# pandekan/tomography_alignment

Measured on AMD Instinct MI355X. Metric: sirt_iterations_per_sec, higher is better.
Workload: dtype f32

## Files before the change

### tomography_alignment_amd/csrc/kernels_tile_gather.hip.h

```cpp

#define GTX 8
#define GTY 8
#define GROWS 14
#define GPITCH 68
#ifndef GWAVES
#define GWAVES 4
#endif
#ifndef GPX
#define GPX 8
#define GPY 12
#endif

#define G_DPP(V, CTRL) __builtin_amdgcn_update_dpp(0, (V), (CTRL), 0xf, 0xf, true)
__device__ __forceinline__ int gwave_min_i32(int v)
{
    v = min(v, G_DPP(v, 0xB1));
    v = min(v, G_DPP(v, 0x4E));
    v = min(v, G_DPP(v, 0x141));
    v = min(v, G_DPP(v, 0x140));
    return min(min(__builtin_amdgcn_readlane(v, 0), __builtin_amdgcn_readlane(v, 16)), min(__builtin_amdgcn_readlane(v, 32), __builtin_amdgcn_readlane(v, 48)));
}
__device__ __forceinline__ int gwave_max_i32(int v)
{
    v = max(v, G_DPP(v, 0xB1));
// ... 54 lines not shown
    for (int c = threadIdx.x; c < n_chunk; c += 64) {
        bool any = false;
        for (int i = max(0, 64 * c - zc_hi - 1); i <= min(ndz - 1, 64 * c + 63 - zc_lo) && !any; ++i) any = flags[i] != 0;
        if (any) first = min(first, c);
    }
#pragma unroll
    for (int o = 32; o > 0; o >>= 1) first = min(first, __shfl_xor(first, o, 64));
    if (threadIdx.x == 0) *shift = first >= n_chunk ? 0 : (GWAVES - first % GWAVES) % GWAVES;
}

template <bool ZERO>
__device__ __forceinline__ void gather_update_store(float *__restrict__ dst, const float *__restrict__ vv, const float *__restrict__ gt, const f32x2 (&acc2)[32],
                                                    int z0, int nz, int positivity, double *__restrict__ err_out)
{
    double err = 0.0;
#define G_UPD1(R, A, V, G)                                  \
    {                                                       \
        float pr_ = (A) * (V);                              \
        asm volatile("" : "+v"(pr_));        \
        R = R + pr_;                                        \
        if (positivity && R < 0.f) R = 0.f;                 \
        if (gt) { const float e_ = (G) - R; err += (double)e_ * (double)e_; } \
    }
    if (z0 + 64 <= nz && (nz & 3) == 0) {
#pragma unroll
        for (int p = 0; p < 64; p += 4) {
            float4 r = *(float4 *)(dst + p);
            const float4 v = *(const float4 *)(vv + p);
            float4 t = {0.f, 0.f, 0.f, 0.f};
            if (gt) t = *(const float4 *)(gt + p);
            G_UPD1(r.x, ZERO ? 0.f : acc2[p / 2].x, v.x, t.x)
            G_UPD1(r.y, ZERO ? 0.f : acc2[p / 2].y, v.y, t.y)
            G_UPD1(r.z, ZERO ? 0.f : acc2[p / 2 + 1].x, v.z, t.z)
            G_UPD1(r.w, ZERO ? 0.f : acc2[p / 2 + 1].y, v.w, t.w)
            *(float4 *)(dst + p) = r;
            __builtin_amdgcn_sched_barrier(0);
        }
    } else {
#pragma unroll
        for (int p = 0; p < 64; ++p)
            if (z0 + p < nz) {
                float r = dst[p];
                G_UPD1(r, ZERO ? 0.f : ((p & 1) ? acc2[p / 2].y : acc2[p / 2].x), vv[p], gt[p])
                dst[p] = r;
            }
    }
#undef G_UPD1
    if (gt) {
        err = wave_sum_d(err);
        if ((threadIdx.x & 63) == 0) atomicAdd(err_out, err);
    }
}

template <int NJ, int UPD>
__global__ __launch_bounds__(GWAVES * 64, 16 / GWAVES) void k_adj_gather_flat(const GfC *__restrict__ cs, int n_proj, const float *__restrict__ proj,
                                                                 float *__restrict__ vol, TomoGeomC g, int xs, int xe, int patched,
                                                                 const unsigned char *__restrict__ zflags, int zc_lo, int zc_hi, const int *__restrict__ zshift,
                                                                 const float *__restrict__ upd_v, const float *__restrict__ upd_gt, int positivity,
                                                                 double *__restrict__ upd_err)
{
    __shared__ __attribute__((aligned(16))) float rows[GWAVES][GROWS * GPITCH];
    __shared__ float4 wtab[3][GWAVES][64];
    const int lane = threadIdx.x & 63;
    const int wv = __builtin_amdgcn_readfirstlane(threadIdx.x >> 6);
    const int ntx = (xe - xs + GTX - 1) / GTX, nty = (g.ny + GTY - 1) / GTY, nzq = (g.nz + 64 * GWAVES - 1) / (64 * GWAVES) + 1;
    int tx, ty, zq;
    if (patched) {
        const int npx = (ntx + GPX - 1) / GPX, npy = (nty + GPY - 1) / GPY;
        const int slot = (int)(blockIdx.x >> 3), patch = (slot / (GPX * GPY)) * 8 + (int)(blockIdx.x & 7), within = slot % (GPX * GPY);
        const int pxy = patch % (npx * npy);
        zq = patch / (npx * npy);
        tx = (pxy / npy) * GPX + within / GPY;
        ty = (pxy % npy) * GPY + within % GPY;
    } else {
        zq = (int)(blockIdx.x % (unsigned)nzq);
        ty = (int)((blockIdx.x / (unsigned)nzq) % (unsigned)nty);
        tx = (int)(blockIdx.x / ((unsigned)nzq * (unsigned)nty));
    }
    const int x0 = xs + tx * GTX, y0 = ty * GTY, z0 = (zq * GWAVES + wv - *zshift) * 64;
    if (tx >= ntx || ty >= nty || zq >= nzq) return;
    bool zlive = z0 >= 0 && z0 < g.nz;
    if (zlive) {
        bool any = false;
        for (int i = z0 - zc_hi - 1 + lane; i <= z0 + 63 - zc_lo; i += 64) any |= i >= 0 && i < g.ndz && zflags[i] != 0;
        zlive = __builtin_amdgcn_ballot_w64(any) != 0;
    }
    __shared__ int wlive[GWAVES];
    if (lane == 0) wlive[wv] = zlive ? 1 : 0;
    __syncthreads();
    int nl = 0, rk = 0;
#pragma unroll
    for (int w = 0; w < GWAVES; ++w) { nl += wlive[w]; rk += w < wv ? wlive[w] : 0; }
#if !defined(__gfx950__) && !defined(__gfx942__) && !defined(__gfx90a__) && defined(__HIP_DEVICE_COMPILE__)
#error "k_adj_gather_flat: divergent exit before barriers is only known to be safe on gfx9-family targets (s_barrier ignores ended waves)"
#endif
    if (UPD && !zlive && z0 >= 0 && z0 < g.nz && (positivity || upd_gt)) {
        const int X = x0 + (lane >> 3), Y = y0 + (lane & 7);
        if (X < xe && Y < g.ny) {
            const size_t o = ((size_t)X * g.ny + Y) * g.nz + z0;
            f32x2 none[32];
            gather_update_store<true>(vol + o, upd_v + o, upd_gt ? upd_gt + o : nullptr, none, z0, g.nz, positivity, upd_err);
        }
    }
    if (!zlive) return;
    const int X = x0 + (lane >> 3), Y = y0 + (lane & 7), Zl = z0 + lane;
    float *wrows = rows[wv];
    const size_t n_det = (size_t)g.ndx * g.ndz;
    const uint32_t pitch4 = (uint32_t)g.ndz * 4u;
    const float two_m32 = 2.3283064365386963e-10f;
    f32x2 acc2[32];
#pragma unroll
    for (int p = 0; p < 32; ++p) acc2[p] = f32x2{0.f, 0.f};

#define G_TABLE(IPX, BUF, SLOT)                                                                                            \
    {                                                                                                                      \
        float4 t4 = {0.f, 0.f, 0.f, 0.f};                                                                                  \
        if ((IPX) < n_proj) {                                                                                              \
            const GfC &ct = cs[IPX];                                                                                       \
            const float qx = (float)X - ct.p0x, qy = (float)Y - ct.p0y;                                                    \
            const float a = ct.m00 * qx + ct.m01 * qy, b = ct.m10 * qx + ct.m11 * qy;                                      \
            const int i0 = (int)ceilf(a - (fabsf(ct.m00) + fabsf(ct.m01) + 5e-3f));                                        \
            const int j0 = (int)ceilf(b - (fabsf(ct.m10) + fabsf(ct.m11) + 5e-3f));                                        \
            int64_t rx = ct.fp0x + (int64_t)i0 * ct.fux + (int64_t)j0 * ct.fdx - ((int64_t)X << 32);                       \
            int64_t ry = ct.fp0y + (int64_t)i0 * ct.fuy + (int64_t)j0 * ct.fdy - ((int64_t)Y << 32);                       \
            float W[3];                                                                                                    \
            _Pragma("unroll") for (int k = 0; k < 3; ++k) {                                                                \
                int64_t sx = rx, sy = ry;                                                                                  \
                float wsum = 0.f;                                                                                          \
                _Pragma("unroll") for (int mth = 0; mth < NJ; ++mth) {                                                     \
                    const int hx = (int)(sx >> 32), hy = (int)(sy >> 32);                                                  \
                    const float fx = (float)(unsigned)sx * two_m32, fy = (float)(unsigned)sy * two_m32;                    \
                                                        \
                    const float wx = select_lanes2(select_lanes(fx, __builtin_amdgcn_ballot_w64(hx == -1)), 1.f - fx, __builtin_amdgcn_ballot_w64(hx == 0)); \
                    const float wy = select_lanes2(select_lanes(fy, __builtin_amdgcn_ballot_w64(hy == -1)), 1.f - fy, __builtin_amdgcn_ballot_w64(hy == 0)); \
                    wsum += select_lanes(wx * wy, __builtin_amdgcn_ballot_w64((unsigned)(j0 + mth) < (unsigned)ct.n));     \
                    sx += ct.fdx; sy += ct.fdy;                                                                            \
                }                                                                                                          \
                W[k] = select_lanes(wsum, __builtin_amdgcn_ballot_w64((unsigned)(i0 + k) < (unsigned)g.ndx));              \
                rx += ct.fux; ry += ct.fuy;                                                                                \
            }                                                                                                              \
            t4.x = __builtin_bit_cast(float, i0); t4.y = W[0]; t4.z = W[1]; t4.w = W[2];                                   \
        }                                                                                                                  \
        wtab[BUF][SLOT][lane] = t4;                                                                                        \
    }
#ifdef TOMO_ABLATE_GATHER_LOADS
#define G_ROW_LOAD(RS, VOFF, SOFF) __int_as_float(0x3f800000 + (int)((VOFF) + (SOFF)))
#else
#define G_ROW_LOAD(RS, VOFF, SOFF) __builtin_bit_cast(float, __builtin_amdgcn_raw_buffer_load_b32((RS), (VOFF), (SOFF), 0))
#endif
    const uint32_t det_bytes = (uint32_t)min((unsigned long long)n_det * 4ull, 0xffffffffull);
#define G_SETUP(IPX, BUF, SLOT)                                                                                            \
    {                                                                                                                      \
        tn = wtab[BUF][SLOT][lane];                                                                                        \
        hit_n = G_HIT(tn);                                                \
        const int i0s = __builtin_bit_cast(int, tn.x);                                                                     \
        ix_lo_n = __builtin_amdgcn_readfirstlane(gwave_min_i32(i0s));                                                      \
        const GfC &cn = cs[IPX];                                                                                           \
        const int iz0 = Zl - cn.zc;                                                                                        \
        const __amdgpu_buffer_rsrc_t srs =                                                                                 \
            __builtin_amdgcn_make_buffer_rsrc((void *)(proj + (size_t)cn.slot * n_det), 0, (int)det_bytes, 0x00020000);    \
        const uint32_t o0 = (uint32_t)min(max(iz0, 0), g.ndz - 1) * 4u;                                                    \
        const uint32_t rowoff = (uint32_t)min(max(ix_lo_n + min(lane, GROWS - 1), 0), g.ndx - 1) * pitch4;                 \
        _Pragma("unroll") for (int r = 0; r < GROWS; ++r)                                                                  \
            y0v[r] = G_ROW_LOAD(srs, o0, (uint32_t)__builtin_amdgcn_readlane((int)rowoff, r));                             \
         \
         \
        if (cn.tau != 0.f) {                                                 \
            const uint32_t oe = (uint32_t)min(max(z0 - cn.zc - 1, 0), g.ndz - 1) * 4u;                                     \
            yedge = __builtin_bit_cast(float, __builtin_amdgcn_raw_buffer_load_b32(srs, rowoff + oe, 0, 0));               \
        }                                                                                                                  \
    }
#define G_ZLERP(MASKED, TAU)                                                                                                      \
    _Pragma("unroll") for (int r = 0; r < GROWS; ++r) {                                                                           \
        float y1 = dpp_shr1_f(y0v[r]);                                             \
        asm("v_writelane_b32 %0, %1, 0" : "+v"(y1) : "s"(__builtin_amdgcn_readlane(__builtin_bit_cast(int, yedge), r)));    \
        const float a0 = (MASKED) ? select_lanes(y0v[r], m0) : y0v[r], a1 = (MASKED) ? select_lanes(y1, m1) : y1;                \
        wrows[r * GPITCH + lane] = fmaf((TAU), a1 - a0, a0);                                                                      \
    }
#define G_STAGE(IPX)                                                                                                       \
    {                                                                                                                      \
        const GfC &cn = cs[IPX];                                                                                           \
        const int iz0 = Zl - cn.zc, iz1 = iz0 - 1;                                                                         \
        const unsigned long long m0 = __builtin_amdgcn_ballot_w64(iz0 >= 0) & __builtin_amdgcn_ballot_w64(iz0 < g.ndz);    \
        const unsigned long long m1 = __builtin_amdgcn_ballot_w64(iz1 >= 0) & __builtin_amdgcn_ballot_w64(iz1 < g.ndz);    \
        if (cn.tau == 0.f) {             \
            if (m0 == ~0ull) {           \
                _Pragma("unroll") for (int r = 0; r < GROWS; ++r) wrows[r * GPITCH + lane] = y0v[r];     \
            } else {                                                                                                       \
                _Pragma("unroll") for (int r = 0; r < GROWS; ++r) wrows[r * GPITCH + lane] = select_lanes(y0v[r], m0);     \
            }                                                                                                              \
        }                                                                                                                  \
        else if ((m0 & m1) == ~0ull) { G_ZLERP(false, cn.tau) }      \
        else { G_ZLERP(true, cn.tau) }                                                                                     \
    }
#define G_HIT(T) (__any((T).y != 0.f || (T).z != 0.f || (T).w != 0.f))
    const int n_grp = (n_proj + nl - 1) / nl;
    int buf = 0;
    float4 t = {0.f, 0.f, 0.f, 0.f};
    int ix_lo = 0;
    bool hit = false;
    if (n_grp > 0) {
        G_TABLE(rk, 0, rk)
        __syncthreads();
        float4 tn;
        int ix_lo_n = 0;
        bool hit_n;
        float y0v[GROWS], yedge = 0.f;
        G_SETUP(0, 0, 0)
        hit = hit_n;
        if (hit) G_STAGE(0)
        t = tn; ix_lo = ix_lo_n;
    }
    for (int grp = 0; grp < n_grp; ++grp) {
        const int nbuf = buf == 2 ? 0 : buf + 1;
        if (grp + 1 < n_grp) G_TABLE((grp + 1) * nl + rk, nbuf, rk)
        __syncthreads();
        const int g0 = grp * nl, g1 = min(n_proj, g0 + nl);
        for (int ip = g0; ip < g1; ++ip) {
            float4 tn = t;
            int ix_lo_n = ix_lo;
            bool hit_n = false;
            float y0v[GROWS], yedge = 0.f;
            const bool more = ip + 1 < n_proj;
            if (more) {
                const bool same = ip + 1 < g1;
                const int sbuf = same ? buf : nbuf, sslot = same ? ip + 1 - g0 : 0;
                G_SETUP(ip + 1, sbuf, sslot)
            }
            if (hit) {
                const int i0 = __builtin_bit_cast(int, t.x);
                const float W0 = t.y, W1 = t.z, W2 = t.w;
                const int slot0 = min(max(i0 - ix_lo, 0), GROWS - 3);
                const float4 *q = (const float4 *)__builtin_assume_aligned(wrows + slot0 * GPITCH, 16);
                float4 n0 = q[0], n1 = q[GPITCH / 4], n2 = q[2 * GPITCH / 4];
#pragma unroll
                for (int p = 0; p < 64; p += 4) {
                    const float4 r0 = n0, r1 = n1, r2 = n2;
                    if (p + 4 < 64) { n0 = q[(p + 4) / 4]; n1 = q[(GPITCH + p + 4) / 4]; n2 = q[(2 * GPITCH + p + 4) / 4]; }
                    acc2[p / 2] = W2 * f32x2{r2.x, r2.y} + (W1 * f32x2{r1.x, r1.y} + (W0 * f32x2{r0.x, r0.y} + acc2[p / 2]));
                    acc2[p / 2 + 1] = W2 * f32x2{r2.z, r2.w} + (W1 * f32x2{r1.z, r1.w} + (W0 * f32x2{r0.z, r0.w} + acc2[p / 2 + 1]));
                    __builtin_amdgcn_sched_barrier(0);
                }
            }
            hit = hit_n;
            if (hit) G_STAGE(ip + 1)
            t = tn; ix_lo = ix_lo_n;
        }
        buf = nbuf;
    }
#undef G_TABLE
#undef G_ROW_LOAD
#undef G_SETUP
#undef G_ZLERP
#undef G_STAGE
#undef G_HIT
    if (UPD) {
        if (X < xe && Y < g.ny) {
            const size_t o = ((size_t)X * g.ny + Y) * g.nz + z0;
            gather_update_store<false>(vol + o, upd_v + o, upd_gt ? upd_gt + o : nullptr, acc2, z0, g.nz, positivity, upd_err);
        }
    } else if (zlive && X < xe && Y < g.ny) {
        float *dst = vol + ((size_t)X * g.ny + Y) * g.nz + z0;
        if (z0 + 64 <= g.nz && (g.nz & 3) == 0) {
#pragma unroll
            for (int p = 0; p < 64; p += 4) {
                float4 v = *(float4 *)(dst + p);
                v.x += acc2[p / 2].x; v.y += acc2[p / 2].y; v.z += acc2[p / 2 + 1].x; v.w += acc2[p / 2 + 1].y;
                *(float4 *)(dst + p) = v;
            }
        } else {
#pragma unroll
            for (int p = 0; p < 64; ++p)
                if (z0 + p < g.nz) dst[p] += (p & 1) ? acc2[p / 2].y : acc2[p / 2].x;
        }
    }
}


#define FGROWS 24
#define FG_NONE (1 << 29)
#ifndef FPG
#define FPG 16
#define FPR 4
#endif
#define FWD_PATCH_MIN 128

__host__ __device__ static inline unsigned long long fg_list_wgs(int n_list, int nrt, int nzq, int patched)
{
    const unsigned long long npg = (unsigned long long)((n_list + 7) / 8);
    if (!patched) return 8ull * ((npg * (unsigned long long)nrt + 7) / 8) * (unsigned long long)nzq;
    const unsigned long long npq = ((npg + FPG - 1) / FPG) * (unsigned long long)((nrt + FPR - 1) / FPR);
    return 8ull * ((npq * (unsigned long long)nzq + 7) / 8) * (unsigned long long)(FPG * FPR);
}

template <int NW, int WALKY>
__device__ __forceinline__ void fwd_gather_flat_body(const GfC *__restrict__ cs, const int *__restrict__ perm, int n_list, unsigned block_id,
                                                     int patched, float *__restrict__ proj, const float *__restrict__ vol, const TomoGeomC &g,
                                                     const unsigned char *__restrict__ vflags, const int *__restrict__ zshift,
                                                     float (*rows)[FGROWS * GPITCH], float4 (*wtab)[GWAVES][64], int (*ltab)[GWAVES][64], int *wlive)
{
    static_assert(NW == 3 || NW == 4, "NW");
    constexpr int SW = FGROWS - NW + 1;
// ... 281 lines not shown
```

### tomography_alignment_amd/csrc/tomo_ctx.h

```cpp
#ifndef TOMO_CTX_H_
#define TOMO_CTX_H_
#include <hip/hip_runtime.h>
#include <rccl/rccl.h>

#include <deque>
#include <map>
#include <string>
#include <vector>

#include "../../include/tomo.h"
#include "tomo_raycore.h"

struct BpC {
    float rp[3][3], ra[3][3], rb[3][3];
    float t[3];
};

struct ProfRec { int64_t n = 0; double ms = 0.0; };
struct ProfPending { std::string name; hipEvent_t e0, e1; };

struct TilePlan {
    bool valid = false;
    bool ok = false;
    std::vector<double> poses;
    int opts = 0;
    double weight_bound = 2.0;
    int n_flat = 0, n_gather = 0;
    double eb_max = 0.0;
    int zc_lo = 0, zc_hi = 0;
    size_t gf_off = 0, fg_off = 0;
    int fg_n[4] = {0, 0, 0, 0};
    bool fg_ok = false;
};

struct ZfKey {
    const void *src = nullptr;
    int nproj = 0, ndz = 0, ndx = 0, nz = 0, zc_lo = 0, zc_hi = 0;
    bool operator==(const ZfKey &o) const
    {
        return src == o.src && nproj == o.nproj && ndz == o.ndz && ndx == o.ndx && nz == o.nz && zc_lo == o.zc_lo && zc_hi == o.zc_hi;
    }
};

struct tomo_ctx {
    int device = 0;
    hipStream_t stream = nullptr;
    bool has_geom = false;
    TomoGeomC g{};
    double vox_pitch[3] = {1, 1, 1};
    float *d_volpad = nullptr;
    size_t volpad_elems = 0;
    size_t volpad_rows = 0;
    bool halo_dirty = true;
    bool wide_rows = false;
    const void *staged_src = nullptr;
    int reuse_staged = 0;
    void *h_stage = nullptr;
    void *d_stage = nullptr;
    size_t stage_bytes = 0;
    TilePlan plan;
    double *d_red = nullptr;
    double *h_red = nullptr;
    size_t red_cap = 0;
    int comm_test_copy_eighths = 0, comm_test_copy_wgs = 0;
    void *d_comm_scratch = nullptr;
    size_t comm_scratch_bytes = 0;
    double *d_red_part = nullptr;
    size_t red_part_cap = 0;
    double *d_acc = nullptr;
    double *h_acc = nullptr;
    int *d_blk = nullptr;
    size_t blk_ints = 0;
    int reuse_sino_flags = 0;
    ZfKey zf_key;
    bool zf_has_cum = false, zf_has_shift = false;
    bool zf_recorded = false;
    float *d_ws = nullptr;
    size_t ws_elems = 0;
    void *csr_data = nullptr, *csr_indices = nullptr, *csr_indptr = nullptr;
    int64_t csr_nnz = 0, csr_rows = 0;
    int csr_value_bytes = 4;
    int fwd_variant = 3;
    int adj_variant = 2;
    int grad_variant = 4;
    int grad_v1_prec = 0;
    int tile_flat = 1;
    int fused_update = 1;
    int adj_flat_gather = 1;
    int fwd_gather_patch = 1;
    int fwd_flat_gather = 1;
    int fwd_flat_ztiles = 2;
    hipEvent_t ev0 = nullptr, ev1 = nullptr;
    bool profile_on = false;
    std::map<std::string, ProfRec> prof;
    std::vector<ProfPending> pending;
    std::vector<hipEvent_t> ev_pool;
    ncclComm_t comm = nullptr;
    hipStream_t comm_stream = nullptr;
    hipEvent_t ev_compute = nullptr, ev_comm = nullptr;
    bool comm_pending = false;
    std::deque<hipEvent_t> comm_done;
    std::deque<hipEvent_t> comm_done_g;
    int comm_test_poison_us = 0;
    std::vector<hipEvent_t> comm_ev_pool;
    int n_ranks = 1, rank = 0;
    std::string err;
};

int tomo_fail(tomo_ctx *ctx, int code, const std::string &msg);

struct TomoRange {
    bool on;
    explicit TomoRange(const char *name);
    ~TomoRange();
    TomoRange(const TomoRange &) = delete;
    TomoRange &operator=(const TomoRange &) = delete;
};
int tomo_roctx_enable(int on);
int tomo_ensure_stage(tomo_ctx *ctx, size_t bytes);
int tomo_ensure_red(tomo_ctx *ctx, size_t n_doubles);
int tomo_ensure_red_part(tomo_ctx *ctx, size_t n_doubles);
int tomo_ensure_ws(tomo_ctx *ctx, size_t n_floats);
int tomo_ensure_blk(tomo_ctx *ctx, size_t n_ints);
struct BlkHead {
    unsigned char *zf;
    int *zcum, *zshift;
    size_t ints;
};
static inline int tomo_blk_head(tomo_ctx *ctx, size_t extra_ints, BlkHead *h)
{
    const size_t zf_ints = ((size_t)ctx->g.ndz + 3) / 4;
    h->ints = zf_ints + (size_t)ctx->g.ndz + 2;
    const int rc = tomo_ensure_blk(ctx, h->ints + extra_ints);
    if (rc) return rc;
    h->zf = (unsigned char *)ctx->d_blk;
    h->zcum = ctx->d_blk + zf_ints;
    h->zshift = h->zcum + ctx->g.ndz + 1;
    return TOMO_OK;
}
struct LiveList {
    int *list;
// ... 40 lines not shown
```

### tomography_alignment_amd/csrc/tomo_ctx.hip

```cpp
#include <string.h>

#include <algorithm>

#include "tomo_ctx.h"

static std::string g_last_error;

int tomo_fail(tomo_ctx *ctx, int code, const std::string &msg)
{
    g_last_error = msg;
    if (ctx) ctx->err = msg;
    return code;
}

extern "C" int tomo_abi_version(void) { return TOMO_ABI_VERSION; }

extern "C" const char *tomo_last_error(const tomo_ctx *ctx) { return ctx ? ctx->err.c_str() : g_last_error.c_str(); }

extern "C" int tomo_device_count(int *n)
{
    if (!n) return tomo_fail(nullptr, TOMO_ERR_ARG, "null n");
    TOMO_HIP(nullptr, hipGetDeviceCount(n));
    return TOMO_OK;
}
// ... 112 lines not shown
}

extern "C" int tomo_sync(tomo_ctx *ctx)
{
    if (!ctx) return tomo_fail(ctx, TOMO_ERR_ARG, "null ctx");
    TOMO_HIP(ctx, hipStreamSynchronize(ctx->stream));
    return TOMO_OK;
}

extern "C" int tomo_ctx_make_current(tomo_ctx *ctx)
{
    if (!ctx) return tomo_fail(ctx, TOMO_ERR_ARG, "null ctx");
    TOMO_HIP(ctx, hipSetDevice(ctx->device));
    return TOMO_OK;
}

extern "C" int tomo_ctx_stream(tomo_ctx *ctx, void **stream)
{
    if (!ctx || !stream) return tomo_fail(ctx, TOMO_ERR_ARG, "tomo_ctx_stream: null argument");
    *stream = reinterpret_cast<void *>(ctx->stream);
    return TOMO_OK;
}

extern "C" int tomo_ctx_set_cu_mask(tomo_ctx *ctx, const uint32_t *mask, int n_words)
{
    if (!ctx || n_words < 0 || (n_words > 0 && !mask)) return tomo_fail(ctx, TOMO_ERR_ARG, "tomo_ctx_set_cu_mask: bad args");
    if (n_words > 0) {
        bool any = false;
        for (int i = 0; i < n_words; ++i) any |= mask[i] != 0;
        if (!any) return tomo_fail(ctx, TOMO_ERR_ARG, "tomo_ctx_set_cu_mask: empty mask (n_words = 0 restores the unrestricted stream)");
    }
    TOMO_HIP(ctx, hipSetDevice(ctx->device));
    TOMO_HIP(ctx, hipStreamSynchronize(ctx->stream));
    hipStream_t s = nullptr;
    if (n_words == 0) TOMO_HIP(ctx, hipStreamCreateWithFlags(&s, hipStreamNonBlocking));
    else TOMO_HIP(ctx, hipExtStreamCreateWithCUMask(&s, (uint32_t)n_words, mask));
    (void)hipStreamDestroy(ctx->stream);
    ctx->stream = s;
    return TOMO_OK;
}

extern "C" int tomo_set_option(tomo_ctx *ctx, const char *key, int value)
{
    if (!ctx || !key) return tomo_fail(ctx, TOMO_ERR_ARG, "bad args");
    if (!strcmp(key, "fwd_variant")) ctx->fwd_variant = value;
    else if (!strcmp(key, "adj_variant")) ctx->adj_variant = value;
    else if (!strcmp(key, "tile_flat")) ctx->tile_flat = value;
    else if (!strcmp(key, "grad_variant")) ctx->grad_variant = value;
    else if (!strcmp(key, "grad_v1_prec")) ctx->grad_v1_prec = value & 3;
    else if (!strcmp(key, "comm_test_poison_us")) ctx->comm_test_poison_us = value;
    else if (!strcmp(key, "comm_test_copy_eighths")) ctx->comm_test_copy_eighths = value < 0 ? 0 : value;
    else if (!strcmp(key, "comm_test_copy_wgs")) ctx->comm_test_copy_wgs = value < 0 ? 0 : value;
    else if (!strcmp(key, "adj_flat_gather")) ctx->adj_flat_gather = value;
    else if (!strcmp(key, "fused_update")) ctx->fused_update = value;
    else if (!strcmp(key, "fwd_flat_ztiles")) ctx->fwd_flat_ztiles = value;
    else if (!strcmp(key, "fwd_flat_gather")) ctx->fwd_flat_gather = value;
    else if (!strcmp(key, "fwd_gather_patch")) {
        if (value < 0 || value > 2) return tomo_fail(ctx, TOMO_ERR_ARG, "fwd_gather_patch: 0, 1 or 2");
        ctx->fwd_gather_patch = value;
    }
    else if (!strcmp(key, "reuse_staged_volume")) ctx->reuse_staged = value;
    else if (!strcmp(key, "reuse_sino_flags")) ctx->reuse_sino_flags = value;
    else if (!strcmp(key, "roctx")) {
        if (tomo_roctx_enable(value)) return tomo_fail(ctx, TOMO_ERR_UNSUPPORTED, "roctx: neither librocprofiler-sdk-roctx.so nor libroctx64.so could be loaded");
    }
    else return tomo_fail(ctx, TOMO_ERR_ARG, std::string("unknown option ") + key);
    return TOMO_OK;
}

int tomo_ensure_stage(tomo_ctx *ctx, size_t bytes)
{
    ctx->plan.valid = false;
    if (bytes <= ctx->stage_bytes) return TOMO_OK;
    TOMO_HIP(ctx, hipStreamSynchronize(ctx->stream));
    if (ctx->d_stage) (void)hipFree(ctx->d_stage);
    if (ctx->h_stage) (void)hipHostFree(ctx->h_stage);
    ctx->d_stage = ctx->h_stage = nullptr;
    ctx->stage_bytes = 0;
    size_t cap = std::max<size_t>(bytes, 1 << 16);
    TOMO_HIP(ctx, hipMalloc(&ctx->d_stage, cap));
    TOMO_HIP(ctx, hipHostMalloc(&ctx->h_stage, cap, hipHostMallocDefault));
    ctx->stage_bytes = cap;
    return TOMO_OK;
}

int tomo_ensure_red(tomo_ctx *ctx, size_t n)
{
    if (n <= ctx->red_cap) return TOMO_OK;
    TOMO_HIP(ctx, hipStreamSynchronize(ctx->stream));
    if (ctx->d_red) (void)hipFree(ctx->d_red);
    if (ctx->h_red) (void)hipHostFree(ctx->h_red);
    ctx->d_red = ctx->h_red = nullptr;
    ctx->red_cap = 0;
    size_t cap = std::max<size_t>(n, 4096);
    TOMO_HIP(ctx, hipMalloc((void **)&ctx->d_red, cap * sizeof(double)));
    TOMO_HIP(ctx, hipHostMalloc((void **)&ctx->h_red, cap * sizeof(double), hipHostMallocDefault));
    ctx->red_cap = cap;
    return TOMO_OK;
}

int tomo_ensure_red_part(tomo_ctx *ctx, size_t n)
{
    if (n <= ctx->red_part_cap) return TOMO_OK;
    TOMO_HIP(ctx, hipStreamSynchronize(ctx->stream));
    if (ctx->d_red_part) (void)hipFree(ctx->d_red_part);
    ctx->d_red_part = nullptr;
// ... 761 lines not shown
```

### tomography_alignment_amd/csrc/tomo_project.hip

```cpp
#include <limits.h>
#include <string.h>

#include <algorithm>
#include <climits>
#include <vector>

#include "tomo_ctx.h"

#include "kernels_ray.hip.h"
#include "kernels_tile.hip.h"
#include "kernels_tile_flat.hip.h"
#include "kernels_tile_gather.hip.h"
#include "kernels_grad.hip.h"

static inline bool grad_pose_is_tilted(const ProjC &c) { return fabs(c.w[0]) + fabs(c.w[1]) > 0.0157; }

static int upload_projc(tomo_ctx *ctx, const double *h_poses, int n, bool with_grad, ProjC **d_pc, GradC **d_gc,
                        const int32_t *h_rows = nullptr, int *n_first = nullptr)
{
    const size_t pc_bytes = sizeof(ProjC) * (size_t)n;
    const size_t gc_off = (pc_bytes + 255) & ~(size_t)255;
    const size_t total = gc_off + (with_grad ? sizeof(GradC) * (size_t)n : 0);
    TOMO_HIP(ctx, hipStreamSynchronize(ctx->stream));
    int rc = tomo_ensure_stage(ctx, total);
// ... 77 lines not shown
    std::vector<int> fg_list[4];
    p.fg_ok = true;
    p.zc_lo = INT_MAX;
    p.zc_hi = INT_MIN;
    for (int i = 0; i < n_proj; ++i) {
        ProjC pc;
        tomo_make_projc(g, h_poses + (size_t)i * TOMO_POSE_STRIDE, pc, nullptr);
        AdjC a;
        double m[3][3], det = 0.0;
        bool fits = true;
        for (int r = 0; r < 3; ++r) {
            a.p0[r] = pc.p0[r]; a.u[r] = pc.u[r]; a.w[r] = pc.w[r]; a.d[r] = pc.d[r];
            m[r][0] = pc.u[r]; m[r][1] = pc.w[r]; m[r][2] = pc.d[r];
            const double lim = 1073741824.0;
            fits = fits && fabs(pc.p0[r]) < lim && fabs(pc.u[r]) * g.ndx < lim && fabs(pc.w[r]) * g.ndz < lim && fabs(pc.d[r]) * pc.n < lim;
            a.fp0[r] = llround(pc.p0[r] * 4294967296.0);
            a.fu[r] = llround(pc.u[r] * 4294967296.0);
            a.fw[r] = llround(pc.w[r] * 4294967296.0);
            a.fd[r] = llround(pc.d[r] * 4294967296.0);
        }
        a.n = pc.n;
        a.slot = i;
        if (!fits) return TOMO_OK;
        if (!invert3(m, a.minv, &det)) return TOMO_OK;
        if (!(pc.w[2] > 0.7 * sqrt(pc.w[0] * pc.w[0] + pc.w[1] * pc.w[1] + pc.w[2] * pc.w[2]))) return TOMO_OK;
        p.weight_bound = std::max(p.weight_bound, 2.0 / fabs(det));
        const bool untilted = a.fw[0] == 0 && a.fw[1] == 0 && a.fw[2] == ((int64_t)1 << 32) && a.fu[2] == 0 && a.fd[2] == 0 &&
                              ctx->tile_flat != 0;
        const double ea = fabs(a.minv[0][0]) + fabs(a.minv[0][1]), eb = fabs(a.minv[2][0]) + fabs(a.minv[2][1]);
        const bool gatherable = untilted && ctx->adj_flat_gather != 0 && ea < 1.45 && eb < 2.99 &&
                                fabs(a.minv[0][2]) < 1e-9 && fabs(a.minv[2][2]) < 1e-9;
        if (gatherable) {
            GfC q;
            q.fp0x = a.fp0[0]; q.fp0y = a.fp0[1]; q.fux = a.fu[0]; q.fuy = a.fu[1]; q.fdx = a.fd[0]; q.fdy = a.fd[1];
            q.m00 = (float)a.minv[0][0]; q.m01 = (float)a.minv[0][1]; q.m10 = (float)a.minv[2][0]; q.m11 = (float)a.minv[2][1];
            q.p0x = (float)a.p0[0]; q.p0y = (float)a.p0[1];
            q.zc = (int32_t)(a.fp0[2] >> 32);
            q.tau = (float)((double)(uint32_t)(a.fp0[2] & 0xffffffffll) / 4294967296.0);
            q.n = a.n; q.slot = a.slot;
            {
                const bool walky = llabs(q.fdx) < llabs(q.fdy);
                const int64_t ads = llabs(walky ? q.fdy : q.fdx), adl = llabs(walky ? q.fdx : q.fdy);
                p.fg_ok = p.fg_ok && (double)ads >= 0.67 * 4294967296.0 && (double)adl < 0.999 * 4294967296.0;
                std::vector<int> &fl = fg_list[2 * (walky ? 1 : 0) + (2 * adl <= ads ? 0 : 1)];
                if (!fl.empty() && fl.back() != (int)gfc.size() - 1)
                    while (fl.size() % 8) fl.push_back(-1);
                fl.push_back((int)gfc.size());
            }
            gath.push_back(a);
            gfc.push_back(q);
            p.eb_max = std::max(p.eb_max, eb);
            p.zc_lo = std::min(p.zc_lo, (int)q.zc);
            p.zc_hi = std::max(p.zc_hi, (int)q.zc);
        } else
            (untilted ? flat : gen).push_back(a);
    }
    AdjC *h = (AdjC *)ctx->h_stage;
    size_t k = 0;
    for (const AdjC &a : gath) h[k++] = a;
    for (const AdjC &a : flat) h[k++] = a;
    for (const AdjC &a : gen) h[k++] = a;
    GfC *hg = (GfC *)((char *)ctx->h_stage + p.gf_off);
    for (size_t i = 0; i < gfc.size(); ++i) hg[i] = gfc[i];
    int *hf = (int *)((char *)ctx->h_stage + p.fg_off);
    size_t fg_total = 0;
    for (int l = 0; l < 4; ++l) {
        for (int v : fg_list[l]) hf[fg_total++] = v;
        p.fg_n[l] = (int)fg_list[l].size();
    }
    if (n_proj) TOMO_HIP(ctx, hipMemcpyAsync(ctx->d_stage, h, p.fg_off + sizeof(int) * fg_total, hipMemcpyHostToDevice, ctx->stream));
    p.n_gather = (int)gath.size();
    p.n_flat = (int)(gath.size() + flat.size());
    p.poses.assign(h_poses, h_poses + n_pose_doubles);
    p.opts = opts;
    p.ok = p.valid = true;
    return TOMO_OK;
}

static inline const AdjC *plan_adjc(const tomo_ctx *ctx) { return (const AdjC *)ctx->d_stage; }
static inline const GfC *plan_gfc(const tomo_ctx *ctx, const TilePlan &p) { return (const GfC *)((const char *)ctx->d_stage + p.gf_off); }
static inline const int *plan_fwd_lists(const tomo_ctx *ctx, const TilePlan &p) { return (const int *)((const char *)ctx->d_stage + p.fg_off); }

static inline dim3 tile_grid(const TomoGeomC &g, int tz = ATZ) { return dim3((g.nz + 1 + tz - 1) / tz, (g.ny + 1 + ATY - 1) / ATY, (g.nx + 1 + ATX - 1) / ATX); }

static int forward_tiles(tomo_ctx *ctx, const double *h_poses, int n_proj, const float *d_vol, float *d_proj, int xt0, int xt1, bool *done,
                         bool whole = false)
{
    const TomoGeomC &g = ctx->g;
    *done = false;
    if (ctx->fwd_variant != 3 || n_proj <= 0) return TOMO_OK;
    dim3 grid = tile_grid(g);
    if (grid.y > 65535 || grid.z > 65535) return TOMO_OK;
    const TilePlan *plan = nullptr;
    int rc = stage_tile_consts(ctx, h_poses, n_proj, &plan);
    if (rc) return rc;
    if (!plan->ok) return TOMO_OK;
    *done = true;
    xt0 = std::max(xt0, 0);
    xt1 = std::min(xt1, (int)grid.z);
    if (xt1 <= xt0) return TOMO_OK;
    grid.z = (unsigned)(xt1 - xt0);
    const AdjC *d_c = plan_adjc(ctx);
    const int n_flat = plan->n_flat;
    size_t flat_ints = 0;
    ctx->zf_key.src = nullptr;
    if (whole && ctx->fwd_flat_gather && plan->n_gather == n_proj && plan->fg_ok && plan->eb_max < 1.49 &&
// ... 145 lines not shown

static int adjoint_tiles(tomo_ctx *ctx, const double *h_poses, int n_proj, const float *d_proj, float *d_vol, int xt0, int xt1, bool *done,
                         const GatherUpd *upd = nullptr)
{
    const TomoGeomC &g = ctx->g;
    const size_t n_det = (size_t)g.ndx * g.ndz;
    dim3 grid = tile_grid(g);
    *done = false;
    if (ctx->adj_variant == 1 || n_proj <= 0 || grid.y > 65535 || grid.z > 65535) return TOMO_OK;
    const TilePlan *plan = nullptr;
    int rc = stage_tile_consts(ctx, h_poses, n_proj, &plan);
    if (rc) return rc;
    if (!plan->ok) return TOMO_OK;
    const int n_flat = plan->n_flat, n_gather = plan->n_gather;
    const int n_xt = (int)grid.z;
    xt0 = std::max(xt0, 0);
    xt1 = std::min(xt1, n_xt);
    if (upd && (n_gather != n_proj || xt0 != 0 || xt1 != n_xt)) return TOMO_OK;
    *done = true;
    if (xt1 <= xt0) return TOMO_OK;
    grid.z = (unsigned)(xt1 - xt0);
    const AdjC *d_c = plan_adjc(ctx);
    const GfC *d_gfc = plan_gfc(ctx, *plan);
    BlkHead head{};
    const size_t n_tile = (size_t)grid.x * grid.y * grid.z;
    if (n_gather > 0 || n_proj > n_flat) {
        rc = tomo_blk_head(ctx, n_proj > n_flat ? LiveList::ints(n_tile) : 0, &head);
        if (rc) return rc;
        const bool want_cum = n_proj > n_flat;
        const bool cached = ctx->zf_key == zf_key_of(ctx, d_proj, n_proj) && (ctx->zf_has_cum || !want_cum) && (ctx->zf_has_shift || n_gather == 0) &&
                            (ctx->reuse_sino_flags || ctx->zf_recorded);
        if (!cached) {
            TOMO_HIP(ctx, hipMemsetAsync(head.zf, 0, (size_t)g.ndz, ctx->stream));
            const long long n_rows = (long long)n_proj * g.ndx;
            const unsigned gy = (unsigned)std::min<long long>(n_rows, 4096);
            TOMO_LAUNCH(ctx, "k_sino_zflags", k_sino_zflags, dim3((unsigned)((g.ndz + 255) / 256), gy), dim3(256), 0, d_proj, n_rows, g.ndz, head.zf);
            rc = tomo_record_zflags(ctx, d_proj, n_proj, want_cum, n_gather > 0, head, "k_sino_zflags", false);
            if (rc) return rc;
        }
    }
    if (n_gather > 0) {
        const int xs = std::max(0, ATX * xt0 - 1), xe = (xt1 == n_xt) ? g.nx : std::min(g.nx, ATX * xt1 - 1);
        if (xe > xs) {
            const int ntx = (xe - xs + GTX - 1) / GTX, nty = (g.ny + GTY - 1) / GTY, nzq = (g.nz + 64 * GWAVES - 1) / (64 * GWAVES) + 1;
            const long long n_patch = (long long)nzq * ((ntx + GPX - 1) / GPX) * ((nty + GPY - 1) / GPY);
            const int patched = n_patch >= 64 ? 1 : 0;
            const long long n_wg = patched ? ((n_patch + 7) / 8) * 8 * (GPX * GPY) : (long long)nzq * ntx * nty;
            if (n_wg >= ((long long)1 << 31)) return tomo_fail(ctx, TOMO_ERR_UNSUPPORTED, "gather adjoint: grid too large");
            const dim3 ggrid((unsigned)n_wg);
            const int zc_lo = plan->zc_lo, zc_hi = plan->zc_hi;
            const float *u_v = upd ? upd->v : nullptr, *u_gt = upd ? upd->gt : nullptr;
            const int u_pos = upd ? upd->positivity : 0;
            if (upd && upd->gt) TOMO_HIP(ctx, hipMemsetAsync(ctx->d_red, 0, sizeof(double), ctx->stream));
#define GATHER_LAUNCH(NJ, UPD)                                                                                                                       \
    TOMO_LAUNCH(ctx, "k_adj_gather_flat", (k_adj_gather_flat<NJ, UPD>), ggrid, dim3(GWAVES * 64), 0, d_gfc, n_gather, d_proj, d_vol, g, xs, xe, patched, \
                (const unsigned char *)head.zf, zc_lo, zc_hi, (const int *)head.zshift, u_v, u_gt, u_pos, ctx->d_red)
            if (plan->eb_max < 1.49) { if (upd) GATHER_LAUNCH(3, 1); else GATHER_LAUNCH(3, 0); }
            else { if (upd) GATHER_LAUNCH(6, 1); else GATHER_LAUNCH(6, 0); }
#undef GATHER_LAUNCH
        }
    }
    if (n_proj == n_gather) return TOMO_OK;
    rc = tomo_ensure_red(ctx, 8);
    if (rc) return rc;
    unsigned *d_absmax = (unsigned *)(ctx->d_red + 4);
    TOMO_HIP(ctx, hipMemsetAsync(d_absmax, 0, sizeof(unsigned), ctx->stream));
    const int64_t n_y = (int64_t)n_det * n_proj;
    TOMO_LAUNCH(ctx, "k_absmax", k_absmax, dim3((unsigned)std::min<int64_t>((n_y + 255) / 256, 2048)), dim3(256), 0, d_proj, n_y, d_absmax);
    if (n_flat > n_gather) {
        dim3 fgrid = tile_grid(g, FTZ);
        fgrid.z = grid.z;
        TOMO_LAUNCH(ctx, "k_adj_tile_flat", k_tile_flat<false>, fgrid, dim3(ADJ_WAVES * 64), 0, d_c + n_gather, n_flat - n_gather, (float *)d_proj,
                    d_vol, g, (const unsigned *)d_absmax, (float)plan->weight_bound, xt0);
    }
    if (n_proj > n_flat) {
        if (n_tile >= (size_t)1 << 30) return tomo_fail(ctx, TOMO_ERR_ARG, "tomo_adjoint: volume too large for the tile list");
        const LiveList live(ctx->d_blk, head.ints, n_tile);
        TOMO_LAUNCH(ctx, "k_sino_zflags", k_tile_adj_live, dim3((unsigned)n_tile), dim3(64), 0, d_c + n_flat, n_proj - n_flat, g, xt0, (int)grid.x,
                    (int)grid.y, (const int *)head.zcum, live.flags);
        TOMO_LAUNCH(ctx, "k_sino_zflags", k_fwd_compact, dim3(1), dim3(1024), 0, (const unsigned char *)live.flags, (int)n_tile, live.list);
        TOMO_LAUNCH(ctx, "k_adj_tile", (k_tile<false, TILE_ADJ_WAVES>), dim3((unsigned)n_tile), dim3(TILE_ADJ_WAVES * 64), 0, d_c + n_flat, n_proj - n_flat, (float *)d_proj, d_vol, g,
                    (const unsigned *)d_absmax, (float)plan->weight_bound, xt0, (const int *)live.list, (int)grid.x, (int)grid.y, (const int *)head.zcum);
    }
    return TOMO_OK;
}

extern "C" int tomo_adjoint(tomo_ctx *ctx, const double *h_poses, int n_proj, const float *d_proj, float *d_vol, int accumulate)
{
    TomoRange roctx_range("tomo_adjoint");
    TOMO_NEED_GEOM(ctx);
    if (!h_poses || !d_vol || !d_proj || n_proj < 0) return tomo_fail(ctx, TOMO_ERR_ARG, "tomo_adjoint: bad args");
    const TomoGeomC &g = ctx->g;
    const size_t n_vox = (size_t)g.nx * g.ny * g.nz;
    if (n_proj == 0) {
        if (!accumulate) TOMO_HIP(ctx, hipMemsetAsync(d_vol, 0, n_vox * sizeof(float), ctx->stream));
        return TOMO_OK;
    }
    if (!accumulate && ctx->adj_variant != 1) TOMO_HIP(ctx, hipMemsetAsync(d_vol, 0, n_vox * sizeof(float), ctx->stream));
    bool done = false;
    int rc = adjoint_tiles(ctx, h_poses, n_proj, d_proj, d_vol, 0, INT_MAX, &done);
    if (rc) return rc;
    if (done) return TOMO_OK;
    return adjoint_atomic(ctx, h_poses, n_proj, d_proj, d_vol, accumulate);
}

extern "C" int tomo_adjoint_update(tomo_ctx *ctx, const double *h_poses, int n_proj, const float *d_res, float *d_rec, const float *d_V, int positivity,
                                   const float *d_gt, double *h_sumsq_err, int *fused)
{
    TomoRange roctx_range("tomo_adjoint_update");
    TOMO_NEED_GEOM(ctx);
    if (!h_poses || !d_res || !d_rec || n_proj < 0 || !fused) return tomo_fail(ctx, TOMO_ERR_ARG, "tomo_adjoint_update: bad args");
// ... 401 lines not shown
```

Baseline: 3.948.

## Add direct-to-LDS buffer-load path for gather adjoint with double-buffered rows

Adds a DMA variant of the flat gather adjoint kernel that loads projection rows straight into LDS via buffer_load_lds, double-buffered across projections. This removes the register round trip and the separate LDS store staging step. The variant is used only when all tilts have zero tau and the angle extent is small, and it uses 13 rows instead of 14. It adds a second LDS buffer, which may cut occupancy, and relies on a barrier and waitcnt scheme whose ordering must be correct.

```diff
diff --git a/tomography_alignment_amd/csrc/kernels_tile_gather.hip.h b/tomography_alignment_amd/csrc/kernels_tile_gather.hip.h
--- a/tomography_alignment_amd/csrc/kernels_tile_gather.hip.h
+++ b/tomography_alignment_amd/csrc/kernels_tile_gather.hip.h
@@ -130,14 +130,18 @@
     }
 }
 
-template <int NJ, int UPD>
+#define GDMA_ROWS 13
+#define GDMA_EA 1.427
+template <int NJ, int UPD, int DMA = 0>
 __global__ __launch_bounds__(GWAVES * 64, 16 / GWAVES) void k_adj_gather_flat(const GfC *__restrict__ cs, int n_proj, const float *__restrict__ proj,
                                                                  float *__restrict__ vol, TomoGeomC g, int xs, int xe, int patched,
                                                                  const unsigned char *__restrict__ zflags, int zc_lo, int zc_hi, const int *__restrict__ zshift,
                                                                  const float *__restrict__ upd_v, const float *__restrict__ upd_gt, int positivity,
                                                                  double *__restrict__ upd_err)
 {
-    __shared__ __attribute__((aligned(16))) float rows[GWAVES][GROWS * GPITCH];
+    static_assert(DMA == 0 || NJ == 3, "the direct-to-LDS loop is built for NJ = 3 only");
+    constexpr int NR = DMA ? GDMA_ROWS : GROWS;
+    __shared__ __attribute__((aligned(16))) float rows[GWAVES][NR * GPITCH];
     __shared__ float4 wtab[3][GWAVES][64];
     const int lane = threadIdx.x & 63;
     const int wv = __builtin_amdgcn_readfirstlane(threadIdx.x >> 6);
@@ -238,8 +242,8 @@
         const __amdgpu_buffer_rsrc_t srs =                                                                                 \
             __builtin_amdgcn_make_buffer_rsrc((void *)(proj + (size_t)cn.slot * n_det), 0, (int)det_bytes, 0x00020000);    \
         const uint32_t o0 = (uint32_t)min(max(iz0, 0), g.ndz - 1) * 4u;                                                    \
-        const uint32_t rowoff = (uint32_t)min(max(ix_lo_n + min(lane, GROWS - 1), 0), g.ndx - 1) * pitch4;                 \
-        _Pragma("unroll") for (int r = 0; r < GROWS; ++r)                                                                  \
+        const uint32_t rowoff = (uint32_t)min(max(ix_lo_n + min(lane, NR - 1), 0), g.ndx - 1) * pitch4;                    \
+        _Pragma("unroll") for (int r = 0; r < NR; ++r)                                                                     \
             y0v[r] = G_ROW_LOAD(srs, o0, (uint32_t)__builtin_amdgcn_readlane((int)rowoff, r));                             \
          \
          \
@@ -249,13 +253,23 @@
         }                                                                                                                  \
     }
 #define G_ZLERP(MASKED, TAU)                                                                                                      \
-    _Pragma("unroll") for (int r = 0; r < GROWS; ++r) {                                                                           \
-        float y1 = dpp_shr1_f(y0v[r]);                                             \
+    _Pragma("unroll") for (int r = 0; r < NR; ++r) {                                                                              \
+        float y1 = dpp_shr1_f(y0v[r]);                                            \
         asm("v_writelane_b32 %0, %1, 0" : "+v"(y1) : "s"(__builtin_amdgcn_readlane(__builtin_bit_cast(int, yedge), r)));    \
         const float a0 = (MASKED) ? select_lanes(y0v[r], m0) : y0v[r], a1 = (MASKED) ? select_lanes(y1, m1) : y1;                \
         wrows[r * GPITCH + lane] = fmaf((TAU), a1 - a0, a0);                                                                      \
     }
-#define G_STAGE(IPX)                                                                                                       \
+#ifdef TOMO_ABLATE_GATHER_STAGE
+#define G_STAGE_COPY                 \
+    {                                                                                                                      \
+        float ysum = y0v[0];                                                                                               \
+        _Pragma("unroll") for (int r = 1; r < NR; ++r) ysum += y0v[r];                                                     \
+        wrows[lane] = ysum;                                                                                                \
+    }
+#else
+#define G_STAGE_COPY _Pragma("unroll") for (int r = 0; r < NR; ++r) wrows[r * GPITCH + lane] = y0v[r];
+#endif
+#define G_STAGE(IPX)                                                                                                      \
     {                                                                                                                      \
         const GfC &cn = cs[IPX];                                                                                           \
         const int iz0 = Zl - cn.zc, iz1 = iz0 - 1;                                                                         \
@@ -263,33 +277,112 @@
         const unsigned long long m1 = __builtin_amdgcn_ballot_w64(iz1 >= 0) & __builtin_amdgcn_ballot_w64(iz1 < g.ndz);    \
         if (cn.tau == 0.f) {             \
             if (m0 == ~0ull) {           \
-                _Pragma("unroll") for (int r = 0; r < GROWS; ++r) wrows[r * GPITCH + lane] = y0v[r];     \
+                G_STAGE_COPY                                          \
             } else {                                                                                                       \
-                _Pragma("unroll") for (int r = 0; r < GROWS; ++r) wrows[r * GPITCH + lane] = select_lanes(y0v[r], m0);     \
+                _Pragma("unroll") for (int r = 0; r < NR; ++r) wrows[r * GPITCH + lane] = select_lanes(y0v[r], m0);        \
             }                                                                                                              \
         }                                                                                                                  \
         else if ((m0 & m1) == ~0ull) { G_ZLERP(false, cn.tau) }      \
         else { G_ZLERP(true, cn.tau) }                                                                                     \
     }
 #define G_HIT(T) (__any((T).y != 0.f || (T).z != 0.f || (T).w != 0.f))
+#define G_ACCUM(WR)                                                                                                        \
+    {                                                                                                                      \
+        const int i0 = __builtin_bit_cast(int, t.x);                                                                       \
+        const float W0 = t.y, W1 = t.z, W2 = t.w;                                                                          \
+        const int slot0 = min(max(i0 - ix_lo, 0), NR - 3);       \
+        const float4 *q = (const float4 *)__builtin_assume_aligned((WR) + slot0 * GPITCH, 16);                             \
+        float4 n0 = q[0], n1 = q[GPITCH / 4], n2 = q[2 * GPITCH / 4];                                                      \
+        _Pragma("unroll") for (int p = 0; p < 64; p += 4) {                                                                \
+            const float4 r0 = n0, r1 = n1, r2 = n2;                                                                        \
+            if (p + 4 < 64) { n0 = q[(p + 4) / 4]; n1 = q[(GPITCH + p + 4) / 4]; n2 = q[(2 * GPITCH + p + 4) / 4]; }       \
+            acc2[p / 2] = W2 * f32x2{r2.x, r2.y} + (W1 * f32x2{r1.x, r1.y} + (W0 * f32x2{r0.x, r0.y} + acc2[p / 2]));      \
+            acc2[p / 2 + 1] = W2 * f32x2{r2.z, r2.w} + (W1 * f32x2{r1.z, r1.w} + (W0 * f32x2{r0.z, r0.w} + acc2[p / 2 + 1])); \
+            __builtin_amdgcn_sched_barrier(0);                                                                             \
+        }                                                                                                                  \
+    }
     const int n_grp = (n_proj + nl - 1) / nl;
     int buf = 0;
     float4 t = {0.f, 0.f, 0.f, 0.f};
     int ix_lo = 0;
     bool hit = false;
-    if (n_grp > 0) {
+    bool reg_loop = true;
+    if constexpr (DMA != 0) {
+        __shared__ __attribute__((aligned(16))) float rows_b[GWAVES][NR * GPITCH];
+        if (z0 - zc_hi >= 0 && z0 + 63 - zc_lo < g.ndz && n_grp > 0) {
+            reg_loop = false;
+            float *const wrows_b = rows_b[wv];
+#define G_DMA_ISSUE(IPX, BUF, SLOT, DST)                                                                                   \
+            {                                                                                                              \
+                tn = wtab[BUF][SLOT][lane];                                                                                \
+                hit_n = G_HIT(tn);                                                                                         \
+                const int i0s = __builtin_bit_cast(int, tn.x);                                                             \
+                ix_lo_n = __builtin_amdgcn_readfirstlane(gwave_min_i32(i0s));                                              \
+                const GfC &cn = cs[IPX];                                                                                   \
+                const __amdgpu_buffer_rsrc_t srs =                                                                         \
+                    __builtin_amdgcn_make_buffer_rsrc((void *)(proj + (size_t)cn.slot * n_det), 0, (int)det_bytes, 0x00020000); \
+                const uint32_t o0 = (uint32_t)min(max(Zl - cn.zc, 0), g.ndz - 1) * 4u;                                     \
+                const uint32_t rowoff = (uint32_t)min(max(ix_lo_n + min(lane, NR - 1), 0), g.ndx - 1) * pitch4;            \
+                _Pragma("unroll") for (int r = 0; r < NR; ++r)                                                             \
+                    __builtin_amdgcn_raw_ptr_buffer_load_lds(srs, (__attribute__((address_space(3))) void *)((DST) + r * GPITCH), 4, (int)o0, \
+                                                             __builtin_amdgcn_readlane((int)rowoff, r), 0, 0);             \
+            }
+#define G_DMA_BARRIER                                                                                                      \
+            {                                                                                                              \
+                asm volatile("s_waitcnt lgkmcnt(0)" ::: "memory");                                                         \
+                __builtin_amdgcn_s_barrier();                                                                              \
+                asm volatile("" ::: "memory");                                                                             \
+            }
+#define G_DMA_PASS(IP, CUR, NXT)                                                                                           \
+            {                                                                                                              \
+                if ((IP) == g1) {                                                                                          \
+                    if ((IP) > 0) buf = nbuf;                                                                              \
+                    nbuf = buf == 2 ? 0 : buf + 1;                                                                         \
+                    g0 = (IP); g1 = min(n_proj, g0 + nl);                                                                  \
+                    if (g0 + nl < n_proj) G_TABLE(g0 + nl + rk, nbuf, rk)                                                  \
+                    G_DMA_BARRIER                                                                                          \
+                }                                                                                                          \
+                {                                                                                                          \
+                    const int ipn = min((IP) + 1, n_proj - 1);                                                             \
+                    const bool same = ipn < g1;                                                                            \
+                    const int sbuf = same ? buf : nbuf, sslot = same ? ipn - g0 : 0;                                       \
+                    G_DMA_ISSUE(ipn, sbuf, sslot, NXT)                                                                     \
+                }                                                                                                          \
+                if (hit) G_ACCUM(CUR)                                                                                      \
+                hit = hit_n; t = tn; ix_lo = ix_lo_n;                                                                      \
+            }
+            G_TABLE(rk, 0, rk)
+            __syncthreads();
+            float4 tn;
+            int ix_lo_n = 0;
+            bool hit_n;
+            G_DMA_ISSUE(0, 0, 0, wrows)
+            hit = hit_n; t = tn; ix_lo = ix_lo_n;
+            int g0 = 0, g1 = 0, nbuf = 0;
+            for (int ip = 0; ip < n_proj; ip += 2) {
+                G_DMA_PASS(ip, wrows, wrows_b)
+                if (ip + 1 >= n_proj) break;
+                G_DMA_PASS(ip + 1, wrows_b, wrows)
+            }
+            asm volatile("s_waitcnt vmcnt(0)" ::: "memory");
+#undef G_DMA_ISSUE
+#undef G_DMA_BARRIER
+#undef G_DMA_PASS
+        }
+    }
+    if (reg_loop && n_grp > 0) {
         G_TABLE(rk, 0, rk)
         __syncthreads();
         float4 tn;
         int ix_lo_n = 0;
         bool hit_n;
-        float y0v[GROWS], yedge = 0.f;
+        float y0v[NR], yedge = 0.f;
         G_SETUP(0, 0, 0)
         hit = hit_n;
         if (hit) G_STAGE(0)
         t = tn; ix_lo = ix_lo_n;
     }
-    for (int grp = 0; grp < n_grp; ++grp) {
+    for (int grp = 0; reg_loop && grp < n_grp; ++grp) {
         const int nbuf = buf == 2 ? 0 : buf + 1;
         if (grp + 1 < n_grp) G_TABLE((grp + 1) * nl + rk, nbuf, rk)
         __syncthreads();
@@ -298,34 +391,22 @@
             float4 tn = t;
             int ix_lo_n = ix_lo;
             bool hit_n = false;
-            float y0v[GROWS], yedge = 0.f;
+            float y0v[NR], yedge = 0.f;
             const bool more = ip + 1 < n_proj;
             if (more) {
                 const bool same = ip + 1 < g1;
                 const int sbuf = same ? buf : nbuf, sslot = same ? ip + 1 - g0 : 0;
                 G_SETUP(ip + 1, sbuf, sslot)
             }
-            if (hit) {
-                const int i0 = __builtin_bit_cast(int, t.x);
-                const float W0 = t.y, W1 = t.z, W2 = t.w;
-                const int slot0 = min(max(i0 - ix_lo, 0), GROWS - 3);
-                const float4 *q = (const float4 *)__builtin_assume_aligned(wrows + slot0 * GPITCH, 16);
-                float4 n0 = q[0], n1 = q[GPITCH / 4], n2 = q[2 * GPITCH / 4];
-#pragma unroll
-                for (int p = 0; p < 64; p += 4) {
-                    const float4 r0 = n0, r1 = n1, r2 = n2;
-                    if (p + 4 < 64) { n0 = q[(p + 4) / 4]; n1 = q[(GPITCH + p + 4) / 4]; n2 = q[(2 * GPITCH + p + 4) / 4]; }
-                    acc2[p / 2] = W2 * f32x2{r2.x, r2.y} + (W1 * f32x2{r1.x, r1.y} + (W0 * f32x2{r0.x, r0.y} + acc2[p / 2]));
-                    acc2[p / 2 + 1] = W2 * f32x2{r2.z, r2.w} + (W1 * f32x2{r1.z, r1.w} + (W0 * f32x2{r0.z, r0.w} + acc2[p / 2 + 1]));
-                    __builtin_amdgcn_sched_barrier(0);
-                }
-            }
+            if (hit) G_ACCUM(wrows)
             hit = hit_n;
             if (hit) G_STAGE(ip + 1)
             t = tn; ix_lo = ix_lo_n;
         }
         buf = nbuf;
     }
+#undef G_ACCUM
+#undef G_STAGE_COPY
 #undef G_TABLE
 #undef G_ROW_LOAD
 #undef G_SETUP
diff --git a/tomography_alignment_amd/csrc/tomo_ctx.h b/tomography_alignment_amd/csrc/tomo_ctx.h
--- a/tomography_alignment_amd/csrc/tomo_ctx.h
+++ b/tomography_alignment_amd/csrc/tomo_ctx.h
@@ -28,6 +28,8 @@
     int n_flat = 0, n_gather = 0;
     double eb_max = 0.0;
     int zc_lo = 0, zc_hi = 0;
+    double ea_max = 0.0;
+    bool tau_zero = true;
     size_t gf_off = 0, fg_off = 0;
     int fg_n[4] = {0, 0, 0, 0};
     bool fg_ok = false;
@@ -87,6 +89,7 @@
     int tile_flat = 1;
     int fused_update = 1;
     int adj_flat_gather = 1;
+    int adj_gather_dma = 1;
     int fwd_gather_patch = 1;
     int fwd_flat_gather = 1;
     int fwd_flat_ztiles = 2;
diff --git a/tomography_alignment_amd/csrc/tomo_ctx.hip b/tomography_alignment_amd/csrc/tomo_ctx.hip
--- a/tomography_alignment_amd/csrc/tomo_ctx.hip
+++ b/tomography_alignment_amd/csrc/tomo_ctx.hip
@@ -188,6 +188,10 @@
     else if (!strcmp(key, "comm_test_copy_eighths")) ctx->comm_test_copy_eighths = value < 0 ? 0 : value;
     else if (!strcmp(key, "comm_test_copy_wgs")) ctx->comm_test_copy_wgs = value < 0 ? 0 : value;
     else if (!strcmp(key, "adj_flat_gather")) ctx->adj_flat_gather = value;
+    else if (!strcmp(key, "adj_gather_dma")) {
+        if (value < 0 || value > 1) return tomo_fail(ctx, TOMO_ERR_ARG, "adj_gather_dma: 0 or 1");
+        ctx->adj_gather_dma = value;
+    }
     else if (!strcmp(key, "fused_update")) ctx->fused_update = value;
     else if (!strcmp(key, "fwd_flat_ztiles")) ctx->fwd_flat_ztiles = value;
     else if (!strcmp(key, "fwd_flat_gather")) ctx->fwd_flat_gather = value;
diff --git a/tomography_alignment_amd/csrc/tomo_project.hip b/tomography_alignment_amd/csrc/tomo_project.hip
--- a/tomography_alignment_amd/csrc/tomo_project.hip
+++ b/tomography_alignment_amd/csrc/tomo_project.hip
@@ -153,6 +153,8 @@
             p.eb_max = std::max(p.eb_max, eb);
             p.zc_lo = std::min(p.zc_lo, (int)q.zc);
             p.zc_hi = std::max(p.zc_hi, (int)q.zc);
+            p.ea_max = std::max(p.ea_max, ea);
+            p.tau_zero = p.tau_zero && q.tau == 0.f;
         } else
             (untilted ? flat : gen).push_back(a);
     }
@@ -404,11 +406,19 @@
             const float *u_v = upd ? upd->v : nullptr, *u_gt = upd ? upd->gt : nullptr;
             const int u_pos = upd ? upd->positivity : 0;
             if (upd && upd->gt) TOMO_HIP(ctx, hipMemsetAsync(ctx->d_red, 0, sizeof(double), ctx->stream));
-#define GATHER_LAUNCH(NJ, UPD)                                                                                                                       \
-    TOMO_LAUNCH(ctx, "k_adj_gather_flat", (k_adj_gather_flat<NJ, UPD>), ggrid, dim3(GWAVES * 64), 0, d_gfc, n_gather, d_proj, d_vol, g, xs, xe, patched, \
-                (const unsigned char *)head.zf, zc_lo, zc_hi, (const int *)head.zshift, u_v, u_gt, u_pos, ctx->d_red)
-            if (plan->eb_max < 1.49) { if (upd) GATHER_LAUNCH(3, 1); else GATHER_LAUNCH(3, 0); }
-            else { if (upd) GATHER_LAUNCH(6, 1); else GATHER_LAUNCH(6, 0); }
+#define GATHER_LAUNCH(NJ, UPD, DMA)                                                                                                                  \
+    TOMO_LAUNCH(ctx, (DMA) ? "k_adj_gather_flat(dma)" : "k_adj_gather_flat", (k_adj_gather_flat<NJ, UPD, DMA>), ggrid, dim3(GWAVES * 64), 0, d_gfc, n_gather, d_proj, \
+                d_vol, g, xs, xe, patched, (const unsigned char *)head.zf, zc_lo, zc_hi, (const int *)head.zshift, u_v, u_gt, u_pos, ctx->d_red)
+#ifdef TOMO_ABLATE_GATHER_STAGE
+            const bool dma = false;
+#else
+            const bool dma = ctx->adj_gather_dma != 0 && plan->tau_zero && plan->ea_max < GDMA_EA;
+#endif
+            if (plan->eb_max < 1.49) {
+                if (dma) { if (upd) GATHER_LAUNCH(3, 1, 1); else GATHER_LAUNCH(3, 0, 1); }
+                else { if (upd) GATHER_LAUNCH(3, 1, 0); else GATHER_LAUNCH(3, 0, 0); }
+            }
+            else { if (upd) GATHER_LAUNCH(6, 1, 0); else GATHER_LAUNCH(6, 0, 0); }
 #undef GATHER_LAUNCH
         }
     }
```

Result: faster. 4.022 (median of 6 runs) (+1.9%).
